# codeslake/RefVSR

Measured on AMD Instinct MI355X. Metric: 4x SR frames/sec (270p->1080p, RefVSR_small_L1), higher is better.
Workload: dtype f16; 1 GPU; config_RefVSR_small_L1 4x SR, 270x480 -> 1080x1920, frame_num=5, steady-state sliding window, n=1 (BASELINE configs[1]); synthetic clip seed 0, seeded random weights 1234; frames_per_rank=20, parallelism=frame-shard x1 (reset-aligned, no collective), window_cache=True, frame_ids=True, pipelined_calls=True, frames_per_call=4, headline_mode=frame groups, pipe_layout=pfm, full=False

## Files before the change

refvsr_amd/csrc/common.h:

```cpp
#pragma once
#include <stdlib.h>
#include <hip/hip_runtime.h>
#include <hip/hip_fp16.h>
#include <stdint.h>
#include <stdio.h>
#include <string.h>
#include <type_traits>
#include <utility>

#include "../../include/refvsr_hip.h"
#include "plan_common.h"

typedef _Float16 f16;
typedef f16 f16x2 __attribute__((ext_vector_type(2)));
typedef f16 f16x4 __attribute__((ext_vector_type(4)));
typedef f16 f16x8 __attribute__((ext_vector_type(8)));
typedef float f32x4 __attribute__((ext_vector_type(4)));
typedef float f32x16 __attribute__((ext_vector_type(16)));

#define RV_HIP(call)                                                                  \
    do {                                                                              \
        hipError_t e_ = (call);                                                       \
        if (e_ != hipSuccess) {                                                       \
            refvsr_set_error("%s failed: %s (%s:%d)", #call, hipGetErrorString(e_), __FILE__, __LINE__); \
// ... 54 lines not shown
    return 0;
}

template <typename Args, typename Launch>
static int rv_resblock_chain(const char* name, int pxb, int min_blob, const void* const* src, int batch, int h, int w, int n,
                             const void* blobs, size_t blob_stride, float act_slope, void* scratch0, void* scratch1, void* const* out,
                             void* stream, Launch launch) {
    RV_CHECK(src && out && blobs && h > 0 && w > 0 && n >= 1 && batch >= 1 && batch <= REFVSR_MAX_MAPS, "%s: bad args", name);
    RV_CHECK(blob_stride >= (size_t)min_blob && blob_stride % 16 == 0 && ((uintptr_t)blobs & 15) == 0,
             "%s: blobs must be 16-byte aligned, stride >= %d", name, min_blob);
    RV_CHECK(act_slope >= 0.f && act_slope <= 1.f, "%s: activation slope must lie in [0, 1]", name);
    RV_CHECK(n == 1 || scratch0, "%s: n >= 2 needs scratch0", name);
    RV_CHECK(n <= 2 || scratch1, "%s: n >= 3 needs scratch1", name);
    const size_t mapb = (size_t)h * w * pxb;
    for (int b = 0; b < batch; ++b) {
        RV_CHECK(src[b] && out[b], "%s: null map pointer (map %d)", name, b);
        for (int c = 0; c < batch; ++c) {
            const unsigned char* s0 = scratch0 ? (const unsigned char*)scratch0 + c * mapb : nullptr;
            const unsigned char* s1 = scratch1 ? (const unsigned char*)scratch1 + c * mapb : nullptr;
            RV_CHECK(src[b] != out[c] && s0 != out[b] && s1 != out[b] && (n < 2 || s0 != src[b]) && (n < 3 || s1 != src[b]) &&
                     (c == b || out[b] != out[c]), "%s: buffers must be distinct", name);
        }
    }
    RV_CHECK(n < 3 || scratch0 != scratch1, "%s: buffers must be distinct", name);
    RV_CHECK((long long)h * w * pxb < (1ll << 31), "%s: map too large for 32-bit offsets", name);
    RV_CHECK(refvsr_init() == 0, "init failed");
    Args a;
    memset(&a, 0, sizeof(a));
    a.h = h; a.w = w; a.act_slope = act_slope; a.batch = batch;
    hipStream_t st = (hipStream_t)stream;
    const unsigned char* cur[REFVSR_MAX_MAPS];
    for (int b = 0; b < batch; ++b) cur[b] = (const unsigned char*)src[b];
    for (int i = 0; i < n; ++i) {
        unsigned char* sc = (unsigned char*)((i & 1) ? scratch1 : scratch0);
        for (int b = 0; b < batch; ++b) {
            a.bsrc[b] = cur[b];
            a.bout[b] = (i == n - 1) ? (unsigned char*)out[b] : sc + b * mapb;
        }
        a.src = a.bsrc[0]; a.out = a.bout[0]; a.blob = (const unsigned char*)blobs + (size_t)i * blob_stride;
        const int rc = launch(a, st);
        if (rc) return rc;
        for (int b = 0; b < batch; ++b) cur[b] = a.bout[b];
    }
    return 0;
}

__device__ __forceinline__ void rv_tile_range(const int n_tiles, const int g, int& t_begin, int& t_end) {
    const int b = (int)blockIdx.x;
    int rank = b;
    if (g >= 8) {
        const int xcd = b & 7;
        rank = b >> 3;
        for (int y = 0; y < xcd; ++y) rank += (g - y + 7) >> 3;
    }
    const unsigned un = (unsigned)n_tiles, ug = (unsigned)g;
    t_begin = (int)(((unsigned)rank * un) / ug);
    t_end = (int)(((unsigned)(rank + 1) * un) / ug);
}

__device__ __forceinline__ int rv_reflect(int i, int n) {
    i = i < 0 ? -i : i;
    return i >= n ? 2 * (n - 1) - i : i;
}

__device__ __forceinline__ float rv_lrelu(float v, float slope) { return v >= 0.f ? v : v * slope; }

__device__ __forceinline__ float rv_linspace_m1p1(int j, int n) {
    const float step = 2.0f / (float)(n - 1);
    return (j < n / 2) ? (-1.0f + step * (float)j) : (1.0f - step * (float)(n - 1 - j));
}

struct WarpCoord { int x0, y0; float w00, w01, w10, w11; bool v00, v01, v10, v11; };

__device__ __forceinline__ WarpCoord warp_coord_uv(const float u, const float v, int hf, int wf, int hin, int win, int y, int x);
__device__ __forceinline__ WarpCoord warp_coord(const float* flow, int hf, int wf, int hin, int win, int y, int x) {
    const size_t fp = (size_t)y * wf + x;
    return warp_coord_uv(flow[fp], flow[(size_t)hf * wf + fp], hf, wf, hin, win, y, x);
}
__device__ __forceinline__ WarpCoord warp_coord_uv(const float u, const float v, int hf, int wf, int hin, int win, int y, int x) {
    const float gx = rv_linspace_m1p1(x, wf) + u / (((float)win - 1.0f) / 2.0f);
    const float gy = rv_linspace_m1p1(y, hf) + v / (((float)hin - 1.0f) / 2.0f);
    const float xs = ((gx + 1.0f) * (float)win - 1.0f) / 2.0f;
    const float ys = ((gy + 1.0f) * (float)hin - 1.0f) / 2.0f;
    const float fx = floorf(xs), fy = floorf(ys);
    const float tx = xs - fx, ty = ys - fy;
    WarpCoord c;
    c.x0 = (int)fminf(fmaxf(fx, -2.0f), (float)win + 1.0f);
    c.y0 = (int)fminf(fmaxf(fy, -2.0f), (float)hin + 1.0f);
    const bool xin0 = c.x0 >= 0 && c.x0 < win, xin1 = c.x0 + 1 >= 0 && c.x0 + 1 < win;
    const bool yin0 = c.y0 >= 0 && c.y0 < hin, yin1 = c.y0 + 1 >= 0 && c.y0 + 1 < hin;
    c.v00 = xin0 && yin0; c.v01 = xin1 && yin0; c.v10 = xin0 && yin1; c.v11 = xin1 && yin1;
    c.w00 = (1.0f - ty) * (1.0f - tx); c.w01 = (1.0f - ty) * tx;
    c.w10 = ty * (1.0f - tx); c.w11 = ty * tx;
    return c;
}

__device__ __forceinline__ uint4 warp_group16(const unsigned char* x, int pixb, int hin, int win, const WarpCoord& c, int goff) {
    float acc[8] = {0, 0, 0, 0, 0, 0, 0, 0};
    auto tap = [&](bool valid, int yy, int xx, float wgt) {
        if (valid) {
            const f16x8 v = *reinterpret_cast<const f16x8*>(x + ((size_t)yy * win + xx) * pixb + goff);
#pragma unroll
            for (int k = 0; k < 8; ++k) acc[k] += wgt * (float)v[k];
        }
    };
    tap(c.v00, c.y0, c.x0, c.w00);
    tap(c.v01, c.y0, c.x0 + 1, c.w01);
    tap(c.v10, c.y0 + 1, c.x0, c.w10);
    tap(c.v11, c.y0 + 1, c.x0 + 1, c.w11);
    union { f16x8 h; uint4 u; } o;
#pragma unroll
    for (int k = 0; k < 8; ++k) o.h[k] = (f16)acc[k];
    return o.u;
}

__device__ __forceinline__ void rv_bilinear_ac_src(int o, int n_in, int n_out, int& i0, int& i1, float& l1) {
#pragma clang fp contract(off)
    const float sc = n_out > 1 ? (float)(n_in - 1) / (float)(n_out - 1) : 0.0f;
    const float x = (float)o * sc;
    i0 = min((int)x, n_in - 1);
    i1 = min(i0 + 1, n_in - 1);
    l1 = x - (float)i0;
}
__device__ __forceinline__ float rv_bilinear_ac2_at(const float* __restrict__ s, int h, int w, int oy, int ox) {
    int y0, y1, x0, x1;
    float ly, lx;
    rv_bilinear_ac_src(oy, h, 2 * h, y0, y1, ly);
    rv_bilinear_ac_src(ox, w, 2 * w, x0, x1, lx);
    const float wy0 = 1.0f - ly, wx0 = 1.0f - lx;
    const float r0 = fmaf(lx, s[(size_t)y0 * w + x1], fmaf(wx0, s[(size_t)y0 * w + x0], 0.0f));
    const float r1 = fmaf(lx, s[(size_t)y1 * w + x1], fmaf(wx0, s[(size_t)y1 * w + x0], 0.0f));
    return fmaf(ly, r1, fmaf(wy0, r0, 0.0f));
}

__device__ __forceinline__ void rv_cubic_taps(float t, float* wgt) {
    const float A = -0.75f;
    float x = t + 1.0f;
    wgt[0] = ((A * x - 5.0f * A) * x + 8.0f * A) * x - 4.0f * A;
    x = t;
    wgt[1] = ((A + 2.0f) * x - (A + 3.0f)) * x * x + 1.0f;
    x = 1.0f - t;
    wgt[2] = ((A + 2.0f) * x - (A + 3.0f)) * x * x + 1.0f;
    x = 2.0f - t;
    wgt[3] = ((A * x - 5.0f * A) * x + 8.0f * A) * x - 4.0f * A;
}
__device__ __forceinline__ void rv_cubic_src(int o, int n_in, float scale, int* idx, float* wgt) {
    const float x = ((float)o + 0.5f) * scale - 0.5f;
    const float fl = floorf(x);
    const int ix = (int)fl;
    rv_cubic_taps(x - fl, wgt);
#pragma unroll
    for (int k = 0; k < 4; ++k) idx[k] = min(max(ix - 1 + k, 0), n_in - 1);
}
__device__ __forceinline__ float rv_bicubic_at(const float* __restrict__ s, int h, int w, int oy, int ox, float sy, float sx) {
    int iy[4], ix[4];
    float wy[4], wx[4];
    rv_cubic_src(oy, h, sy, iy, wy);
    rv_cubic_src(ox, w, sx, ix, wx);
    float acc = 0.0f;
#pragma unroll
    for (int j = 0; j < 4; ++j) {
        float r = 0.0f;
        const float* row = s + (size_t)iy[j] * w;
#pragma unroll
        for (int i = 0; i < 4; ++i) r = fmaf(wx[i], row[ix[i]], r);
        acc = fmaf(wy[j], r, acc);
    }
    return acc;
}

__device__ __forceinline__ void rv_store_result(void* out, const size_t e, const float v, const int fmt) {
    const int f = fmt & REFVSR_RESULT_FMT_MASK;
    if (f == REFVSR_RESULT_F32) reinterpret_cast<float*>(out)[e] = v;
    else if (f == REFVSR_RESULT_F16) reinterpret_cast<f16*>(out)[e] = (f16)v;
    else reinterpret_cast<unsigned char*>(out)[e] = (unsigned char)__float2int_rn(v * 255.0f);
}
__host__ __device__ __forceinline__ size_t rv_result_index(const int fmt, const int c, const int y, const int x, const int h, const int w) {
    return (fmt & REFVSR_RESULT_HWC) ? ((size_t)y * w + x) * 3 + c : ((size_t)c * h + y) * w + x;
}
static inline bool rv_result_fmt_ok(const int fmt) {
    return fmt >= 0 && (fmt & ~(REFVSR_RESULT_FMT_MASK | REFVSR_RESULT_HWC)) == 0 && (fmt & REFVSR_RESULT_FMT_MASK) <= REFVSR_RESULT_U8;
}

__device__ __forceinline__ float rv_fold1(const float a) {
    const unsigned u = __float_as_uint(a);
    const auto pr = __builtin_amdgcn_permlane32_swap(u, u, false, false);
    const unsigned x0 = pr[0], x1 = pr[1];
    return __uint_as_float(x0) + __uint_as_float(x1);
}

__device__ __forceinline__ int rv_pix16(int n) { return (n < 4 || n >= 12) ? ((n & 7) << 1) : (((n - 4) << 1) | 1); }
```

refvsr_amd/csrc/conv24.hip:

```cpp
#include "common.h"
#include "fixed_plan.h"

struct C24Args {
    const unsigned char* src0; const unsigned char* src1; unsigned char* out;
    const unsigned char* blob; const unsigned char* mul; const unsigned char* res;
    int h, w, tiles_x, n_tiles, grid;
    float act_slope, post_slope;
    const float* conf_a; const float* conf_b;
    const float* cw0; const float* cb0;
    float* conf_max;
    int ch, cw;
    float slope0;
    const float* base_lr; int bh, bw; float base_step;
    int out_fmt;
    int batch, tpm;
    const unsigned char* bsrc0[REFVSR_MAX_MAPS]; const unsigned char* bsrc1[REFVSR_MAX_MAPS]; unsigned char* bout[REFVSR_MAX_MAPS];
    const unsigned char* bmul[REFVSR_MAX_MAPS]; const unsigned char* bres[REFVSR_MAX_MAPS];
    const float* bconf_a[REFVSR_MAX_MAPS]; const float* bconf_b[REFVSR_MAX_MAPS]; float* bconf_max[REFVSR_MAX_MAPS];
};

template <int COUT, int NCG0, int NCG1, int NWV, int TH, int WPS, int SHUF = 0, int CONF = 0, int HALF = 0, int MM = 0, int WF = 0>
__global__ __launch_bounds__(NWV * 64) __attribute__((amdgpu_waves_per_eu(WPS, WPS))) void conv24_kernel(C24Args p) {
    static_assert(WF == 0 || COUT != 3, "output head: one fragment in either format");
    static_assert(HALF == 0 || (COUT == 24 && SHUF == 0 && CONF == 0), "channel-half variant: 24 computed channels per workgroup");
    static_assert(MM == 0 || (HALF == 0 && COUT != 3), "multi-map variant");
    static_assert(SHUF == 0 || (COUT == 48 && (SHUF == 24 || SHUF == 48) && NCG0 * 8 == SHUF && NCG1 == 0), "pixel-shuffle variant");
    static_assert(CONF == 0 || (NCG0 == 2 && NCG1 == 0 && SHUF == 0), "confidence variant: 16-channel single source");
    constexpr int NCG = NCG0 + NCG1, PS = NCG | 1, PXB = PS * 16, ROWB = C24_XW * PXB;
    constexpr int S = c24_steps(NCG), NPAT = c24_npat(NCG);
    constexpr int NF = c24_nf(COUT, WF);
    constexpr int NM = COUT == 24 ? 2 : COUT == 3 ? 1 : COUT / 16;
    constexpr int BIASB = COUT == 48 ? 256 : 128;
    constexpr int WB = S * NF * 1024, BIAS = WB, XT = WB + BIASB;
    constexpr int NT = NWV * 64, T = 2 * TH / NWV;
    constexpr int C24_TH = TH, C24_XH = TH + 2, C24_NPX = C24_XH * C24_XW;
    constexpr int NCH = C24_NPX * NCG, KCH = (NCH + NT - 1) / NT;
    constexpr int PIXB0 = NCG0 * 16, PIXB1 = NCG1 * 16;
    constexpr int OPX = HALF ? 96 : COUT * 2;
    static_assert((COUT == 3 || COUT == 24 || COUT == 32 || COUT == 48) && S > 0 && T >= 1 && T * NWV == 2 * TH, "unsupported shape");
    static_assert(COUT != 3 || (NCG1 == 0 && SHUF == 0 && CONF == 0), "output head: single source");
    extern __shared__ __attribute__((aligned(16))) unsigned char smem[];

    asm volatile("" :: "s"(p.src0), "s"(p.src1), "s"(p.out), "s"(p.blob), "s"(p.mul), "s"(p.res), "s"(p.h), "s"(p.w), "s"(p.tiles_x),
                 "s"(p.n_tiles), "s"(p.grid), "s"(p.act_slope), "s"(p.post_slope));
    const int tid = threadIdx.x;
    const int lane = tid & 63;
    const int wave = __builtin_amdgcn_readfirstlane(tid >> 6);

    {
        constexpr int NPC = WB / 1024;
        const unsigned char* g = p.blob + ((SHUF || HALF) ? (int)blockIdx.y * (WB + BIASB) : 0) + lane * 16;
#pragma unroll
        for (int j = 0; j < (NPC + NWV - 1) / NWV; ++j) {
            const int c = wave + j * NWV;
            if (c < NPC)
                __builtin_amdgcn_global_load_lds((const __attribute__((address_space(1))) void*)(g + c * 1024),
                                                 (__attribute__((address_space(3))) void*)(smem + c * 1024), 16, 0, 0);
        }
        if (wave == NPC % NWV && lane < BIASB / 16)
            __builtin_amdgcn_global_load_lds((const __attribute__((address_space(1))) void*)(g + NPC * 1024),
                                             (__attribute__((address_space(3))) void*)(smem + NPC * 1024), 16, 0, 0);
    }

    if constexpr (HALF != 0) {
        const int zoff = (int)blockIdx.y * 48;
        p.out += zoff;
        if (p.mul) p.mul += zoff;
        if (p.res) p.res += zoff;
    }
    const int rowp = p.w;
    unsigned xg[KCH], xl[KCH];
    unsigned xs1 = 0;
#pragma unroll
    for (int k = 0; k < KCH; ++k) {
        const int i = min(tid + k * NT, NCH - 1);
        const int px = i / NCG, cg = i - px * NCG;
        const int r = px / C24_XW, c = px - r * C24_XW;
        const bool s1 = cg >= NCG0;
        xg[k] = (unsigned)((r * rowp + c) * (s1 ? PIXB1 : PIXB0) + (s1 ? cg - NCG0 : cg) * 16);
        xl[k] = (unsigned)(XT + px * PXB + cg * 16);
        xs1 |= s1 ? (1u << k) : 0u;
    }
    uint4 xv[KCH];
    auto x_fetch = [&](const int tf) {
        int t = tf;
        const unsigned char* s0p = p.src0;
        const unsigned char* s1p = p.src1;
        if constexpr (MM != 0) {
            const int bm = (int)((unsigned)tf / (unsigned)p.tpm);
            t = tf - bm * p.tpm;
            s0p = p.bsrc0[bm];
            if constexpr (NCG1 != 0) s1p = p.bsrc1[bm];
        }
        const int tyi = t / p.tiles_x;
        const int ty0 = tyi * C24_TH, tx0 = (t - tyi * p.tiles_x) * C24_TW;
        const bool interior = ty0 >= 1 && ty0 + C24_TH + 1 <= p.h && tx0 >= 1 && tx0 + C24_TW + 1 <= p.w;
        const long long org = (long long)(ty0 - 1) * p.w + (tx0 - 1);
        const unsigned char* b0 = s0p + org * PIXB0;
        const unsigned char* b1 = NCG1 ? s1p + org * PIXB1 : b0;
        if (interior) {
#pragma unroll
            for (int k = 0; k < KCH; ++k)
                xv[k] = *reinterpret_cast<const uint4*>((NCG1 && ((xs1 >> k) & 1) ? b1 : b0) + xg[k]);
        } else {
            int tide = tid;
            asm volatile("" : "+v"(tide));
#pragma unroll
            for (int k = 0; k < KCH; ++k) {
                const int i = min(tide + k * NT, NCH - 1);
                const int px = i / NCG, cg = i - px * NCG;
                const int r = px / C24_XW, c = px - r * C24_XW;
                const int iy = ty0 - 1 + r, ix = tx0 - 1 + c;
                const bool ok = (unsigned)iy < (unsigned)p.h && (unsigned)ix < (unsigned)p.w;
                const bool s1 = cg >= NCG0;
                const unsigned pix = (unsigned)(min(max(iy, 0), p.h - 1) * p.w + min(max(ix, 0), p.w - 1));
                const unsigned char* g = s1 ? s1p + pix * PIXB1 + (cg - NCG0) * 16 : s0p + pix * PIXB0 + cg * 16;
                uint4 v = *reinterpret_cast<const uint4*>(g);
                const unsigned keep = ok ? 0xffffffffu : 0u;
                v.x &= keep; v.y &= keep; v.z &= keep; v.w &= keep;
                xv[k] = v;
            }
        }
    };
    auto x_park = [&]() {
#pragma unroll
        for (int k = 0; k < KCH; ++k)
            if (k * NT + NT <= NCH || tid + k * NT < NCH) *reinterpret_cast<uint4*>(smem + xl[k]) = xv[k];
    };
    constexpr int PTH = TH + 4, PTW = C24_XW + 2;
    constexpr int PT = XT + C24_NPX * PXB, CW0 = PT + 2 * PTH * PTW * 4, CB0 = CW0 + 18 * 16 * 4;
    if constexpr (CONF != 0) {
        float* wl0 = reinterpret_cast<float*>(smem + CW0);
        for (int i = tid; i < 18 * 16; i += NT) {
            const int co = i & 15, tap = i >> 4;
            wl0[i] = p.cw0[(co * 2 + tap / 9) * 9 + tap % 9];
        }
        if (tid < 16) reinterpret_cast<float*>(smem + CB0)[tid] = p.cb0[tid];
    }
    auto conf_stage = [&](const int tf) {
        int t = tf;
        const float* cap = p.conf_a;
        const float* cbp = p.conf_b;
        float* cmp_ = p.conf_max;
        if constexpr (MM != 0) {
            const int bm = (int)((unsigned)tf / (unsigned)p.tpm);
            t = tf - bm * p.tpm;
            cap = p.bconf_a[bm]; cbp = p.bconf_b[bm];
            if (p.conf_max) cmp_ = p.bconf_max[bm];
        }
        const int tyi = t / p.tiles_x;
        const int ty0 = tyi * C24_TH, tx0 = (t - tyi * p.tiles_x) * C24_TW;
        float* pt = reinterpret_cast<float*>(smem + PT);
        for (int i = tid; i < 2 * PTH * PTW; i += NT) {
            const int c = i / (PTH * PTW), rem = i - c * (PTH * PTW);
            const int r = rem / PTW, cc = rem - r * PTW;
            const int y = ty0 - 2 + r, x = tx0 - 2 + cc;
            float v = 0.0f;
            if ((unsigned)y < (unsigned)p.h && (unsigned)x < (unsigned)p.w) {
                const float* src = c ? cbp : cap;
                if constexpr (CONF == 1) v = src[(size_t)y * p.cw + x];
                else v = fminf(fmaxf(rv_bicubic_at(src, p.ch, p.cw, y, x, 0.5f, 0.5f), 0.0f), 1.0f);
            }
            pt[i] = v;
        }
        __syncthreads();
        const float* wl0 = reinterpret_cast<const float*>(smem + CW0);
        const float* bl0 = reinterpret_cast<const float*>(smem + CB0);
#pragma unroll
        for (int k = 0; k < KCH; ++k) {
            const int i = tid + k * NT;
            if (i < NCH) {
                const int px = i >> 1, cg = i & 1;
                const int r = px / C24_XW, c = px - r * C24_XW;
                const int iy = ty0 - 1 + r, ix = tx0 - 1 + c;
                uint4 v = make_uint4(0u, 0u, 0u, 0u);
                if ((unsigned)iy < (unsigned)p.h && (unsigned)ix < (unsigned)p.w) {
                    float acc[8] = {0.f, 0.f, 0.f, 0.f, 0.f, 0.f, 0.f, 0.f};
#pragma unroll
                    for (int ci = 0; ci < 2; ++ci)
#pragma unroll
                        for (int ky = 0; ky < 3; ++ky)
#pragma unroll
                            for (int kx = 0; kx < 3; ++kx) {
                                const float xv = pt[ci * (PTH * PTW) + (r + ky) * PTW + (c + kx)];
                                const f32x4 w0 = *reinterpret_cast<const f32x4*>(wl0 + (ci * 9 + ky * 3 + kx) * 16 + cg * 8);
                                const f32x4 w1 = *reinterpret_cast<const f32x4*>(wl0 + (ci * 9 + ky * 3 + kx) * 16 + cg * 8 + 4);
                                acc[0] = fmaf(xv, w0[0], acc[0]); acc[1] = fmaf(xv, w0[1], acc[1]);
                                acc[2] = fmaf(xv, w0[2], acc[2]); acc[3] = fmaf(xv, w0[3], acc[3]);
                                acc[4] = fmaf(xv, w1[0], acc[4]); acc[5] = fmaf(xv, w1[1], acc[5]);
                                acc[6] = fmaf(xv, w1[2], acc[6]); acc[7] = fmaf(xv, w1[3], acc[7]);
                            }
                    union { f16x8 h; uint4 u; } o;
#pragma unroll
                    for (int j = 0; j < 8; ++j) o.h[j] = (f16)rv_lrelu(acc[j] + bl0[cg * 8 + j], p.slope0);
                    v = o.u;
                }
                *reinterpret_cast<uint4*>(smem + XT + px * PXB + cg * 16) = v;
            }
        }
        if constexpr (CONF == 1) {
            if (p.conf_max) {
                for (int i = tid; i < C24_TH * C24_TW; i += NT) {
                    const int r = i / C24_TW, c = i - r * C24_TW;
                    const int y = ty0 + r, x = tx0 + c;
                    if (y < p.h && x < p.w)
                        cmp_[(size_t)y * p.w + x] = fmaxf(pt[(r + 2) * PTW + c + 2], pt[PTH * PTW + (r + 2) * PTW + c + 2]);
                }
            }
        }
    };
    int tl, k_hi;
    rv_tile_range(p.n_tiles, p.grid, tl, k_hi);
    if constexpr (CONF == 0) { if (tl < k_hi) x_fetch(tl); }
    __builtin_amdgcn_sched_barrier(0);

    const int q = lane >> 4;
    const int lp = rv_pix16(lane & 15);
    const int la = lane * 16;
    const int g0w = wave * T;
#define RW(t) ((g0w + (t)) >> 1)
#define CG(t) ((g0w + (t)) & 1)
    auto sel4 = [&](const int v0, const int v1, const int v2, const int v3) { return q == 0 ? v0 : q == 1 ? v1 : q == 2 ? v2 : v3; };
    int pb[T];
#pragma unroll
    for (int t = 0; t < T; ++t)
        pb[t] = XT + RW(t) * ROWB + (CG(t) * 16 + lp) * PXB +
                sel4(c24_off(NCG, 0, 0), c24_off(NCG, 0, 1), c24_off(NCG, 0, 2), c24_off(NCG, 0, 3)) - c24_off(NCG, 0, 0);
    int pd[NPAT];
#pragma unroll
    for (int pp = 0; pp < NPAT; ++pp) {
        const int s = c24_pat_step(NCG, pp);
        pd[pp] = (sel4(c24_off(NCG, s, 0), c24_off(NCG, s, 1), c24_off(NCG, s, 2), c24_off(NCG, s, 3)) - c24_off(NCG, s, 0)) -
                 (sel4(c24_off(NCG, 0, 0), c24_off(NCG, 0, 1), c24_off(NCG, 0, 2), c24_off(NCG, 0, 3)) - c24_off(NCG, 0, 0));
    }
    const int rowb_o = p.w * OPX;
    const unsigned oo = (unsigned)(lp * OPX + q * 8);

    if constexpr (CONF == 0) { if (tl < k_hi) x_park(); }
    __syncthreads();

    for (; tl < k_hi; ++tl) {
        const bool has_next = tl + 1 < k_hi;
        if constexpr (CONF != 0) {
            conf_stage(tl);
            __syncthreads();
        }
        int tm = tl;
        unsigned char* outp = p.out;
        const unsigned char* mulp = p.mul;
        const unsigned char* resp = p.res;
        if constexpr (MM != 0) {
            const int bm = (int)((unsigned)tl / (unsigned)p.tpm);
            tm = tl - bm * p.tpm;
            outp = p.bout[bm];
            if (p.mul) mulp = p.bmul[bm];
            if (p.res) resp = p.bres[bm];
        }
        const int tyi = tm / p.tiles_x;
        const int ty0 = tyi * C24_TH, tx0 = (tm - tyi * p.tiles_x) * C24_TW;
        const bool interior = ty0 >= 1 && ty0 + C24_TH + 1 <= p.h && tx0 >= 1 && tx0 + C24_TW + 1 <= p.w;
        const long long oorg = ((long long)ty0 * p.w + tx0) * OPX;
        f16x4 mv[NM][T], rv[NM][T];
        bool okt[T];
#pragma unroll
        for (int t = 0; t < T; ++t) {
            okt[t] = true;
            if (!interior) {
                int lpe = lp;
                asm volatile("" : "+v"(lpe));
                okt[t] = ty0 + RW(t) < p.h && tx0 + CG(t) * 16 + lpe < p.w;
            }
            const unsigned eo = (unsigned)(RW(t) * rowb_o) + oo + CG(t) * 16 * OPX;
#pragma unroll
            for (int m = 0; m < NM; ++m) {
                mv[m][t] = rv[m][t] = (f16x4){(f16)0.f, (f16)0.f, (f16)0.f, (f16)0.f};
                const bool lane_ok = okt[t] && (COUT != 24 || m == 0 || q < 2);
                if constexpr (COUT == 24) {
                    if (p.mul && lane_ok) mv[m][t] = *reinterpret_cast<const f16x4*>(mulp + oorg + eo + 32 * m);
                    if (p.res && lane_ok) rv[m][t] = *reinterpret_cast<const f16x4*>(resp + oorg + eo + 32 * m);
                }
                (void)lane_ok;
            }
        }
        if constexpr (CONF == 0) { if (has_next) x_fetch(tl + 1); }

        f32x4 acc[NM][T];
#pragma unroll
        for (int m = 0; m < NM; ++m) {
            const f32x4 bv = *reinterpret_cast<const f32x4*>(smem + BIAS + m * 64 + q * 16);
#pragma unroll
            for (int t = 0; t < T; ++t) acc[m][t] = bv;
        }
        {
            uint4 fa[2][NF], fb[2][T];
            auto load = [&](auto sc, uint4 (&af)[NF], uint4 (&bf)[T]) {
                constexpr int s = decltype(sc)::value;
                constexpr int pp = c24_pat(NCG, s);
                constexpr int imm = c24_off(NCG, s, 0);
#pragma unroll
                for (int f = 0; f < NF; ++f) af[f] = *reinterpret_cast<const uint4*>(smem + (s * NF + f) * 1024 + la);
#pragma unroll
                for (int t = 0; t < T; ++t) {
                    if constexpr (pp == 0) bf[t] = *reinterpret_cast<const uint4*>(smem + pb[t] + imm);
                    else bf[t] = *reinterpret_cast<const uint4*>(smem + pb[t] + pd[pp] + imm);
                }
            };
            auto mfma = [&](const uint4 (&af)[NF], const uint4 (&bf)[T]) {
                if constexpr (WF == 1) {
#pragma unroll
                    for (int m = 0; m < NM; ++m) {
                        const f16x8 av = *reinterpret_cast<const f16x8*>(&af[m]);
#pragma unroll
                        for (int t = 0; t < T; ++t)
                            acc[m][t] = __builtin_amdgcn_mfma_f32_16x16x32_f16(av, *reinterpret_cast<const f16x8*>(&bf[t]), acc[m][t], 0, 0, 0);
                    }
                } else if constexpr (COUT == 24) {
                    const f16x8 a_hi = *reinterpret_cast<const f16x8*>(&af[0]);
                    const f16x8 a_lo = *reinterpret_cast<const f16x8*>(&af[1]);
                    const f16x8 a_mx = *reinterpret_cast<const f16x8*>(&af[2]);
#pragma unroll
                    for (int t = 0; t < T; ++t) acc[0][t] = __builtin_amdgcn_mfma_f32_16x16x32_f16(a_hi, *reinterpret_cast<const f16x8*>(&bf[t]), acc[0][t], 0, 0, 0);
#pragma unroll
                    for (int t = 0; t < T; ++t) acc[1][t] = __builtin_amdgcn_mfma_f32_16x16x32_f16(a_mx, *reinterpret_cast<const f16x8*>(&bf[t]), acc[1][t], 0, 0, 0);
#pragma unroll
                    for (int t = 0; t < T; ++t) acc[0][t] = __builtin_amdgcn_mfma_f32_16x16x32_f16(a_lo, *reinterpret_cast<const f16x8*>(&bf[t]), acc[0][t], 0, 0, 0);
                } else if constexpr (COUT == 3) {
                    const f16x8 a_w = *reinterpret_cast<const f16x8*>(&af[0]);
#pragma unroll
                    for (int t = 0; t < T; ++t) acc[0][t] = __builtin_amdgcn_mfma_f32_16x16x32_f16(a_w, *reinterpret_cast<const f16x8*>(&bf[t]), acc[0][t], 0, 0, 0);
                } else {
#pragma unroll
                    for (int h = 0; h < 2; ++h)
#pragma unroll
                        for (int m = 0; m < NM; ++m) {
                            const f16x8 av = *reinterpret_cast<const f16x8*>(&af[2 * m + h]);
#pragma unroll
                            for (int t = 0; t < T; ++t)
                                acc[m][t] = __builtin_amdgcn_mfma_f32_16x16x32_f16(av, *reinterpret_cast<const f16x8*>(&bf[t]), acc[m][t], 0, 0, 0);
                        }
                }
            };
            if constexpr (NF <= 4) {
                load(std::integral_constant<int, 0>{}, fa[0], fb[0]);
                rv_static_for([&](auto sc) {
                    constexpr int s = decltype(sc)::value;
                    if constexpr (s + 1 < S) load(std::integral_constant<int, s + 1>{}, fa[(s + 1) & 1], fb[(s + 1) & 1]);
                    __builtin_amdgcn_sched_barrier(0);
                    mfma(fa[s & 1], fb[s & 1]);
                }, std::make_integer_sequence<int, S>{});
            } else {
                load(std::integral_constant<int, 0>{}, fa[0], fb[0]);
                rv_static_for([&](auto sc) {
                    constexpr int s = decltype(sc)::value;
                    __builtin_amdgcn_sched_barrier(0);
                    mfma(fa[0], fb[0]);
                    __builtin_amdgcn_sched_barrier(0);
                    if constexpr (s + 1 < S) load(std::integral_constant<int, s + 1>{}, fa[0], fb[0]);
                }, std::make_integer_sequence<int, S>{});
            }
        }
        if (has_next) {
            __syncthreads();
            if constexpr (CONF == 0) x_park();
        }
        if constexpr (COUT == 3) {
            const size_t plane_b = (size_t)p.bh * p.bw;
#pragma unroll
            for (int t = 0; t < T; ++t) {
                const f32x4 y = acc[0][t];
                const float s0 = rv_fold1(y[0]), s1 = rv_fold1(y[1]), s2 = rv_fold1(y[2]);
                const int srcl = lane & 15;
                const float v0 = __shfl(s0, srcl), v1 = __shfl(s1, srcl), v2 = __shfl(s2, srcl);
                const float v = q == 0 ? v0 : q == 1 ? v1 : v2;
                int lpe = lp;
                if (!interior) asm volatile("" : "+v"(lpe));
                const int oy = ty0 + RW(t), ox = tx0 + CG(t) * 16 + lpe;
                if (q < 3 && oy < p.h && ox < p.w) {
                    const float b = fminf(fmaxf(rv_bicubic_at(p.base_lr + q * plane_b, p.bh, p.bw, oy, ox, p.base_step, p.base_step), 0.0f), 1.0f);
                    rv_store_result(outp, rv_result_index(p.out_fmt, q, oy, ox, p.h, p.w), fminf(fmaxf(v + b, 0.0f), 1.0f), p.out_fmt);
                }
            }
        } else if constexpr (SHUF != 0) {
            const int z = (int)blockIdx.y;
            const unsigned w2 = 2u * (unsigned)p.w;
#pragma unroll
            for (int t = 0; t < T; ++t) {
                int lpe = lp;
                if (!interior) asm volatile("" : "+v"(lpe));
                const unsigned oy = (unsigned)(ty0 + RW(t)), ox = (unsigned)(tx0 + CG(t) * 16 + lpe);
#pragma unroll
                for (int m = 0; m < NM; ++m) {
                    const int r0 = 16 * m + 4 * q;
                    const int dx = SHUF == 24 ? (r0 >= 24 ? 1 : 0) : (z & 1);
                    const int dy = SHUF == 24 ? z : (z >> 1);
                    const int ch0 = SHUF == 24 ? r0 - 24 * dx : r0;
                    f32x4 y = acc[m][t];
                    if (p.act_slope != 1.0f) {
#pragma unroll
                        for (int i = 0; i < 4; ++i) y[i] = fmaxf(y[i], y[i] * p.act_slope);
                    }
                    const f16x4 o = {(f16)y[0], (f16)y[1], (f16)y[2], (f16)y[3]};
                    if (okt[t])
                        *reinterpret_cast<f16x4*>(outp + ((2u * oy + dy) * w2 + 2u * ox + dx) * (unsigned)(SHUF * 2) + ch0 * 2) = o;
                }
            }
        } else
        {
            unsigned char* ob = outp + oorg;
#pragma unroll
            for (int t = 0; t < T; ++t) {
                unsigned char* d = ob + (unsigned)(RW(t) * rowb_o) + oo + CG(t) * 16 * OPX;
#pragma unroll
                for (int m = 0; m < NM; ++m) {
                    f32x4 y = acc[m][t];
                    if constexpr (COUT == 24) {
                        if (WF == 0 && m == 1) y = (f32x4){rv_fold1(y[0]), rv_fold1(y[1]), rv_fold1(y[2]), rv_fold1(y[3])};
                    } else {
                        const unsigned eo = (unsigned)(RW(t) * rowb_o) + oo + CG(t) * 16 * OPX;
                        if (p.mul && okt[t]) mv[m][t] = *reinterpret_cast<const f16x4*>(mulp + oorg + eo + 32 * m);
                        if (p.res && okt[t]) rv[m][t] = *reinterpret_cast<const f16x4*>(resp + oorg + eo + 32 * m);
                    }
                    if (p.act_slope != 1.0f) {
#pragma unroll
                        for (int i = 0; i < 4; ++i) y[i] = fmaxf(y[i], y[i] * p.act_slope);
                    }
                    if (p.mul) {
#pragma unroll
                        for (int i = 0; i < 4; ++i) y[i] *= (float)mv[m][t][i];
                    }
                    if (p.res) {
#pragma unroll
                        for (int i = 0; i < 4; ++i) y[i] += (float)rv[m][t][i];
                    }
                    if (p.post_slope != 1.0f) {
#pragma unroll
                        for (int i = 0; i < 4; ++i) y[i] = fmaxf(y[i], y[i] * p.post_slope);
                    }
                    const f16x4 o = {(f16)y[0], (f16)y[1], (f16)y[2], (f16)y[3]};
                    if (okt[t] && (COUT != 24 || m == 0 || q < 2)) *reinterpret_cast<f16x4*>(d + 32 * m) = o;
                }
            }
        }
        if constexpr (CONF == 0) { if (has_next) __syncthreads(); }
    }
#undef RW
#undef CG
}

template <int COUT, int NCG0, int NCG1, int NWV, int TH, int WPS, int SHUF, int CONF, int HALF, int MM, int WF>
static int launch_c24(C24Args& a, const C24Plan& p, hipStream_t st) {
    constexpr int NZ = c24_nz(SHUF, HALF), LDS = c24_lds(COUT, NCG0 + NCG1, TH, CONF, WF);
    static_assert(LDS <= 160 * 1024, "LDS budget");
    static RvLaunchCap lc = {};
    int cap;
    if (int rc = rv_launch_cap(lc, &conv24_kernel<COUT, NCG0, NCG1, NWV, TH, WPS, SHUF, CONF, HALF, MM, WF>, NWV * 64, LDS, LDS, st, &cap, NZ)) return rc;
    a.tiles_x = p.tiles_x; a.tpm = p.tpm; a.n_tiles = p.n_tiles;
    a.grid = a.n_tiles < cap ? a.n_tiles : cap;
    hipLaunchKernelGGL((conv24_kernel<COUT, NCG0, NCG1, NWV, TH, WPS, SHUF, CONF, HALF, MM, WF>), dim3(a.grid, NZ), dim3(NWV * 64), LDS, st, a);
    RV_LAUNCH_CHECK();
    return 0;
}

static const C24Knobs& c24_knobs() {
    static const C24Knobs knobs = c24_knobs_from_env();
    return knobs;
}

static const char* c24_no_kernel(const C24Plan& p) { return p.no_twin ? p.no_twin : "conv24: no kernel for this plan"; }

static int c24_dispatch(C24Args& a, const C24Plan& p, void* stream) {
    switch (p.key()) {
#define RV_C24_CASE(...) case c24_variant_key(__VA_ARGS__): return launch_c24<__VA_ARGS__>(a, p, (hipStream_t)stream);
        RV_C24_VARIANTS(RV_C24_CASE)
#undef RV_C24_CASE
    }
    RV_CHECK(false, "%s", c24_no_kernel(p));
    return 1;
}

extern "C" int refvsr_conv24_variant(int op, int x0, int x1, int mm, int wf, int batch, int h, int w, long long* key, int* n_tiles, int* lds) {
    RV_CHECK(key != nullptr, "conv24_variant: null key");
    RV_CHECK(op >= C24_CONV24 && op <= C24_CONV_LAST && (mm == 0 || mm == 1) && (wf == 0 || wf == 1) && h > 0 && w > 0, "conv24_variant: bad args");
    C24Plan p;
    if (int rc = c24_plan((C24Op)op, x0, x1, mm, wf, mm ? batch : 1, h, w, c24_knobs(), &p)) return rc;
    bool listed = false;
    switch (p.key()) {
#define RV_C24_CASE(...) case c24_variant_key(__VA_ARGS__):
        RV_C24_VARIANTS(RV_C24_CASE) listed = !p.no_twin;
#undef RV_C24_CASE
    }
    RV_CHECK(listed, "%s", c24_no_kernel(p));
    *key = p.key();
    if (n_tiles) *n_tiles = p.n_tiles;
    if (lds) *lds = p.lds;
    return 0;
}

extern "C" int refvsr_conv24_supported(int c0, int c1) { return c24_supported(C24_CONV24, c0, c1); }
extern "C" int refvsr_conv48_supported(int c0, int c1) { return c24_supported(C24_CONV48, c0, c1); }
extern "C" int refvsr_conv32_supported(int c0, int c1) { return c24_supported(C24_CONV32, c0, c1); }
extern "C" int refvsr_conv_shuffle2_supported(int c) { return c24_supported(C24_SHUFFLE2, c, 0); }

extern "C" int refvsr_conv24_blob_bytes(int c0, int c1) { return refvsr_conv24_supported(c0, c1) ? c24_blob_bytes(24, (c0 + c1) / 8, 0) : -1; }
extern "C" int refvsr_conv32_blob_bytes(int c0, int c1) { return refvsr_conv32_supported(c0, c1) ? c24_blob_bytes(32, (c0 + c1) / 8, 0) : -1; }
extern "C" int refvsr_conv48_blob_bytes(int c0, int c1) {
    if (!refvsr_conv48_supported(c0, c1)) return -1;
    return c0 == 48 && c1 == 48 ? c24_nz(0, 1) * c24_blob_bytes(24, 12, 0) : c24_blob_bytes(48, (c0 + c1) / 8, 0);
}
extern "C" int refvsr_conv_shuffle2_blob_bytes(int c) { return refvsr_conv_shuffle2_supported(c) ? c24_nz(c, 0) * c24_blob_bytes(48, c / 8, 0) : -1; }
extern "C" int refvsr_conv24_f16w_blob_bytes(int c0, int c1) { return refvsr_conv24_supported(c0, c1) ? c24_blob_bytes(24, (c0 + c1) / 8, 1) : -1; }
extern "C" int refvsr_conv32_f16w_blob_bytes(int c0, int c1) { return refvsr_conv32_supported(c0, c1) ? c24_blob_bytes(32, (c0 + c1) / 8, 1) : -1; }
extern "C" int refvsr_conv_shuffle2_f16w_blob_bytes(int c) { return c == 24 ? c24_nz(c, 0) * c24_blob_bytes(48, c / 8, 1) : -1; }

extern "C" int refvsr_conv24_kblock(int ncg, int s, int q) {
    if (c24_steps(ncg) == 0 || s < 0 || s >= c24_steps(ncg) || q < 0 || q > 3) return -2;
    return c24_kblock(ncg, s, q);
}

static int c24_fill(C24Args& a, const char* who, int cout, const void* src0, const void* src1, int c1, int h, int w, const void* blob,
                    float act_slope, const void* mul, const void* res, float post_slope, void* out) {
    RV_CHECK(src0 && out && blob && h > 0 && w > 0, "%s: bad args", who);
    RV_CHECK((c1 == 0) == (src1 == nullptr), "%s: src1 / c1 mismatch", who);
    RV_CHECK(((uintptr_t)blob & 15) == 0, "%s: blob must be 16-byte aligned", who);
    RV_CHECK(act_slope >= 0.f && act_slope <= 1.f && post_slope >= 0.f && post_slope <= 1.f, "%s: activation slopes must lie in [0, 1]", who);
    RV_CHECK(src0 != out && src1 != out, "%s: in-place operation is not supported", who);
    RV_CHECK((long long)h * w * cout * 2 < (1ll << 31), "%s: map too large for 32-bit offsets", who);
    RV_CHECK(refvsr_init() == 0, "init failed");
    memset(&a, 0, sizeof(a));
    a.src0 = (const unsigned char*)src0; a.src1 = (const unsigned char*)src1; a.out = (unsigned char*)out;
    a.blob = (const unsigned char*)blob; a.mul = (const unsigned char*)mul; a.res = (const unsigned char*)res;
    a.h = h; a.w = w; a.act_slope = act_slope; a.post_slope = post_slope;
    return 0;
}

static int c24_fill_maps(C24Args& a, const char* who, int cout, const void* const* src0, const void* const* src1, int c1, int batch,
                         int h, int w, const void* blob, float act_slope, const void* const* mul, const void* const* res,
                         float post_slope, void* const* out) {
    if (c24_fill(a, who, cout, src0[0], src1 ? src1[0] : nullptr, c1, h, w, blob, act_slope, mul ? mul[0] : nullptr,
                 res ? res[0] : nullptr, post_slope, out[0])) return 1;
    a.batch = batch;
    for (int b = 0; b < batch; ++b) {
        RV_CHECK(src0[b] && out[b] && (!src1 || src1[b]) && (!mul || mul[b]) && (!res || res[b]), "%s: null map pointer (map %d)", who, b);
        for (int c = 0; c < batch; ++c)
            RV_CHECK(src0[c] != out[b] && (!src1 || src1[c] != out[b]) && (c == b || out[c] != out[b]), "%s: in-place operation is not supported", who);
        a.bsrc0[b] = (const unsigned char*)src0[b]; a.bsrc1[b] = src1 ? (const unsigned char*)src1[b] : nullptr;
        a.bout[b] = (unsigned char*)out[b];
        a.bmul[b] = mul ? (const unsigned char*)mul[b] : nullptr; a.bres[b] = res ? (const unsigned char*)res[b] : nullptr;
    }
    return 0;
}
#define C24_OPT(p) ((p) ? &(p) : nullptr)

static int c24_conv24(int wf, int mm, const void* const* src0, int c0, const void* const* src1, int c1, int batch, int h, int w, const void* blob,
                      float act_slope, const void* const* mul, const void* const* res, float post_slope, void* const* out, void* stream) {
    const char* who = mm ? "conv24_batch" : "conv24";
    C24Plan p;
    C24Args a;
    if (c24_plan(C24_CONV24, c0, c1, mm, wf, batch, h, w, c24_knobs(), &p)) return 1;
    RV_CHECK(src0 && out, "%s: 1..%d maps per launch", who, REFVSR_MAX_MAPS);
    RV_CHECK(!mm || (c1 == 0) == (src1 == nullptr), "%s: src1 / c1 mismatch", who);
    if (c24_fill_maps(a, who, 24, src0, src1, c1, batch, h, w, blob, act_slope, mul, res, post_slope, out)) return 1;
    return c24_dispatch(a, p, stream);
}
#define C24_CONV_ARGS const void* src0, int c0, const void* src1, int c1, int h, int w, const void* blob, float act_slope, \
                      const void* mul, const void* res, float post_slope, void* out, void* stream
#define C24_CONV_BATCH_ARGS const void* const* src0, int c0, const void* const* src1, int c1, int batch, int h, int w, const void* blob, \
                            float act_slope, const void* const* mul, const void* const* res, float post_slope, void* const* out, void* stream
#define C24_CONV_PASS(WF) c24_conv24(WF, 0, &src0, c0, C24_OPT(src1), c1, 1, h, w, blob, act_slope, C24_OPT(mul), C24_OPT(res), post_slope, &out, stream)
#define C24_CONV_BATCH_PASS(WF) c24_conv24(WF, 1, src0, c0, src1, c1, batch, h, w, blob, act_slope, mul, res, post_slope, out, stream)
extern "C" int refvsr_conv24(C24_CONV_ARGS) { return C24_CONV_PASS(0); }
extern "C" int refvsr_conv24_f16w(C24_CONV_ARGS) { return C24_CONV_PASS(1); }
extern "C" int refvsr_conv24_batch(C24_CONV_BATCH_ARGS) { return C24_CONV_BATCH_PASS(0); }
extern "C" int refvsr_conv24_batch_f16w(C24_CONV_BATCH_ARGS) { return C24_CONV_BATCH_PASS(1); }

static int c24_conv_single(C24Op op, const char* who, int cout, int wf, C24_CONV_ARGS) {
    C24Plan p;
    C24Args a;
    if (c24_plan(op, c0, c1, 0, wf, 1, h, w, c24_knobs(), &p)) return 1;
    if (c24_fill(a, who, cout, src0, src1, c1, h, w, blob, act_slope, mul, res, post_slope, out)) return 1;
    return c24_dispatch(a, p, stream);
}
#define C24_CONV_SINGLE(OP, WHO, COUT, WF) c24_conv_single(OP, WHO, COUT, WF, src0, c0, src1, c1, h, w, blob, act_slope, mul, res, post_slope, out, stream)
extern "C" int refvsr_conv32(C24_CONV_ARGS) { return C24_CONV_SINGLE(C24_CONV32, "conv32", 32, 0); }
extern "C" int refvsr_conv32_f16w(C24_CONV_ARGS) { return C24_CONV_SINGLE(C24_CONV32, "conv32", 32, 1); }
extern "C" int refvsr_conv48(C24_CONV_ARGS) { return C24_CONV_SINGLE(C24_CONV48, "conv48", 48, 0); }

static int c24_conv_shuffle2(int wf, int mm, const void* const* src, int batch, int c, int h, int w, const void* blobs, float act_slope,
                             void* const* out, void* stream) {
    const char* who = mm ? "conv_shuffle2_batch" : "conv_shuffle2";
    C24Plan p;
    C24Args a;
    if (c24_plan(C24_SHUFFLE2, c, 0, mm, wf, batch, h, w, c24_knobs(), &p)) return 1;
    RV_CHECK(src && out, "%s: 1..%d maps per launch", who, REFVSR_MAX_MAPS);
    if (c24_fill_maps(a, who, 4 * c, src, nullptr, 0, batch, h, w, blobs, act_slope, nullptr, nullptr, 1.0f, out)) return 1;
    return c24_dispatch(a, p, stream);
}
// ... 60 lines not shown
```

Baseline: 236.4 frames/s.

## Prefetch confidence inputs across tiles and factor bicubic upsample in conv24 confidence stage

The confidence variant of the fused conv24 kernel now prefetches the raw confidence window for the next tile into registers during the current tile's MMA work, then parks it in LDS. The bicubic 2x upsample reuses separable row sums with fixed even/odd tap weights instead of a full 16-tap evaluation per output. The first-layer 2->16 conv is restructured so each thread computes a run of 3 pixels by 4 output channels with double-buffered operand loads. The changes aim to hide global-load latency and cut redundant interpolation and LDS traffic, at the cost of more registers and extra barriers per tile in the confidence path.

```diff
diff --git a/refvsr_amd/csrc/common.h b/refvsr_amd/csrc/common.h
--- a/refvsr_amd/csrc/common.h
+++ b/refvsr_amd/csrc/common.h
@@ -230,21 +230,23 @@
 #pragma unroll
     for (int k = 0; k < 4; ++k) idx[k] = min(max(ix - 1 + k, 0), n_in - 1);
 }
+template <class F>
+__device__ __forceinline__ float rv_cubic_dot(const float* wgt, F v) {
+    float r = 0.0f;
+#pragma unroll
+    for (int k = 0; k < 4; ++k) r = fmaf(wgt[k], v(k), r);
+    return r;
+}
+template <class F>
+__device__ __forceinline__ float rv_bicubic_eval(const float* wy, const float* wx, F tap) {
+    return rv_cubic_dot(wy, [&](const int j) { return rv_cubic_dot(wx, [&](const int i) { return tap(j, i); }); });
+}
 __device__ __forceinline__ float rv_bicubic_at(const float* __restrict__ s, int h, int w, int oy, int ox, float sy, float sx) {
     int iy[4], ix[4];
     float wy[4], wx[4];
     rv_cubic_src(oy, h, sy, iy, wy);
     rv_cubic_src(ox, w, sx, ix, wx);
-    float acc = 0.0f;
-#pragma unroll
-    for (int j = 0; j < 4; ++j) {
-        float r = 0.0f;
-        const float* row = s + (size_t)iy[j] * w;
-#pragma unroll
-        for (int i = 0; i < 4; ++i) r = fmaf(wx[i], row[ix[i]], r);
-        acc = fmaf(wy[j], r, acc);
-    }
-    return acc;
+    return rv_bicubic_eval(wy, wx, [&](const int j, const int i) { return (s + (size_t)iy[j] * w)[ix[i]]; });
 }
 
 __device__ __forceinline__ void rv_store_result(void* out, const size_t e, const float v, const int fmt) {
diff --git a/refvsr_amd/csrc/conv24.hip b/refvsr_amd/csrc/conv24.hip
--- a/refvsr_amd/csrc/conv24.hip
+++ b/refvsr_amd/csrc/conv24.hip
@@ -137,70 +137,156 @@
         }
         if (tid < 16) reinterpret_cast<float*>(smem + CB0)[tid] = p.cb0[tid];
     }
-    auto conf_stage = [&](const int tf) {
+    constexpr int RWH = TH / 2 + 6, RWW = C24_TW / 2 + 6, RWS = (RWW + 3) / 4;
+    constexpr int NRAW = CONF == 2 ? 2 * RWH * RWW : 2 * PTH * PTW, KRAW = (NRAW + NT - 1) / NT;
+    static_assert(CONF == 0 || (PS == 3 && 2 * RWH * RWS <= C24_NPX && TH % 2 == 0), "confidence variant: raw window in slot 2 of the x tile");
+    auto raw_off = [](const int c, const int r, const int cc) { return XT + 32 + ((c * RWH + r) * RWS + (cc >> 2)) * PXB + (cc & 3) * 4; };
+    float craw[KRAW];
+    unsigned cok = 0;
+    auto conf_fetch = [&](const int tf) {
+        int tide = tid;
+        asm volatile("" : "+v"(tide));
         int t = tf;
         const float* cap = p.conf_a;
         const float* cbp = p.conf_b;
+        if constexpr (MM != 0) {
+            const int bm = (int)((unsigned)tf / (unsigned)p.tpm);
+            t = tf - bm * p.tpm;
+            cap = p.bconf_a[bm]; cbp = p.bconf_b[bm];
+        }
+        const int tyi = t / p.tiles_x;
+        const int ty0 = tyi * C24_TH, tx0 = (t - tyi * p.tiles_x) * C24_TW;
+        cok = 0;
+#pragma unroll
+        for (int k = 0; k < KRAW; ++k) {
+            const int i = min(tide + k * NT, NRAW - 1);
+            if constexpr (CONF == 1) {
+                const int c = i / (PTH * PTW), rem = i - c * (PTH * PTW);
+                const int r = rem / PTW, cc = rem - r * PTW;
+                const int y = ty0 - 2 + r, x = tx0 - 2 + cc;
+                cok |= ((unsigned)y < (unsigned)p.h && (unsigned)x < (unsigned)p.w) ? (1u << k) : 0u;
+                craw[k] = (c ? cbp : cap)[(size_t)min(max(y, 0), p.h - 1) * p.cw + min(max(x, 0), p.w - 1)];
+            } else {
+                const int c = i / (RWH * RWW), rem = i - c * (RWH * RWW);
+                const int r = rem / RWW, cc = rem - r * RWW;
+                const int y = min(max(ty0 / 2 - 3 + r, 0), p.ch - 1), x = min(max(tx0 / 2 - 3 + cc, 0), p.cw - 1);
+                craw[k] = (c ? cbp : cap)[(size_t)y * p.cw + x];
+            }
+        }
+    };
+    auto conf_park = [&]() {
+        int tide = tid;
+        asm volatile("" : "+v"(tide));
+#pragma unroll
+        for (int k = 0; k < KRAW; ++k) {
+            const int i = tide + k * NT;
+            if (k * NT + NT <= NRAW || i < NRAW) {
+                if constexpr (CONF == 1) {
+                    reinterpret_cast<float*>(smem + PT)[i] = ((cok >> k) & 1) ? craw[k] : 0.0f;
+                } else {
+                    const int c = i / (RWH * RWW), rem = i - c * (RWH * RWW);
+                    const int r = rem / RWW, cc = rem - r * RWW;
+                    *reinterpret_cast<float*>(smem + raw_off(c, r, cc)) = craw[k];
+                }
+            }
+        }
+    };
+    auto conf_stage = [&](const int tf) {
+        int tide = tid;
+        asm volatile("" : "+v"(tide));
+        int t = tf;
         float* cmp_ = p.conf_max;
         if constexpr (MM != 0) {
             const int bm = (int)((unsigned)tf / (unsigned)p.tpm);
             t = tf - bm * p.tpm;
-            cap = p.bconf_a[bm]; cbp = p.bconf_b[bm];
             if (p.conf_max) cmp_ = p.bconf_max[bm];
         }
         const int tyi = t / p.tiles_x;
         const int ty0 = tyi * C24_TH, tx0 = (t - tyi * p.tiles_x) * C24_TW;
         float* pt = reinterpret_cast<float*>(smem + PT);
-        for (int i = tid; i < 2 * PTH * PTW; i += NT) {
-            const int c = i / (PTH * PTW), rem = i - c * (PTH * PTW);
-            const int r = rem / PTW, cc = rem - r * PTW;
-            const int y = ty0 - 2 + r, x = tx0 - 2 + cc;
-            float v = 0.0f;
-            if ((unsigned)y < (unsigned)p.h && (unsigned)x < (unsigned)p.w) {
-                const float* src = c ? cbp : cap;
-                if constexpr (CONF == 1) v = src[(size_t)y * p.cw + x];
-                else v = fminf(fmaxf(rv_bicubic_at(src, p.ch, p.cw, y, x, 0.5f, 0.5f), 0.0f), 1.0f);
-            }
-            pt[i] = v;
-        }
-        __syncthreads();
+        if constexpr (CONF == 2) {
+            float wev[4], wod[4];
+            rv_cubic_taps(0.75f, wev);
+            rv_cubic_taps(0.25f, wod);
+            if (tide < PTH * PTW) {
+                const int c = tide / (PTH / 2 * PTW), rem = tide - c * (PTH / 2 * PTW);
+                const int k = rem / PTW, cc = rem - k * PTW;
+                const int y = ty0 - 2 + 2 * k, x = tx0 - 2 + cc, rx = (cc + 1) >> 1;
+                float wx[4];
+#pragma unroll
+                for (int i = 0; i < 4; ++i) wx[i] = (cc & 1) ? wod[i] : wev[i];
+                int co[4];
+#pragma unroll
+                for (int i = 0; i < 4; ++i) co[i] = raw_off(0, 0, rx + i) - raw_off(0, 0, 0);
+                float rs[5];
+#pragma unroll
+                for (int j = 0; j < 5; ++j) {
+                    const unsigned char* row = smem + raw_off(c, k + j, 0);
+                    rs[j] = rv_cubic_dot(wx, [&](const int i) { return *reinterpret_cast<const float*>(row + co[i]); });
+                }
+                float v0 = rv_cubic_dot(wev, [&](const int j) { return rs[j]; });
+                float v1 = rv_cubic_dot(wod, [&](const int j) { return rs[j + 1]; });
+                const bool xin = (unsigned)x < (unsigned)p.w;
+                v0 = (xin && (unsigned)y < (unsigned)p.h) ? fminf(fmaxf(v0, 0.0f), 1.0f) : 0.0f;
+                v1 = (xin && (unsigned)(y + 1) < (unsigned)p.h) ? fminf(fmaxf(v1, 0.0f), 1.0f) : 0.0f;
+                pt[c * (PTH * PTW) + 2 * k * PTW + cc] = v0;
+                pt[c * (PTH * PTW) + (2 * k + 1) * PTW + cc] = v1;
+            }
+            __syncthreads();
+        }
         const float* wl0 = reinterpret_cast<const float*>(smem + CW0);
         const float* bl0 = reinterpret_cast<const float*>(smem + CB0);
-#pragma unroll
-        for (int k = 0; k < KCH; ++k) {
-            const int i = tid + k * NT;
-            if (i < NCH) {
-                const int px = i >> 1, cg = i & 1;
-                const int r = px / C24_XW, c = px - r * C24_XW;
-                const int iy = ty0 - 1 + r, ix = tx0 - 1 + c;
-                uint4 v = make_uint4(0u, 0u, 0u, 0u);
-                if ((unsigned)iy < (unsigned)p.h && (unsigned)ix < (unsigned)p.w) {
-                    float acc[8] = {0.f, 0.f, 0.f, 0.f, 0.f, 0.f, 0.f, 0.f};
-#pragma unroll
-                    for (int ci = 0; ci < 2; ++ci)
-#pragma unroll
-                        for (int ky = 0; ky < 3; ++ky)
-#pragma unroll
-                            for (int kx = 0; kx < 3; ++kx) {
-                                const float xv = pt[ci * (PTH * PTW) + (r + ky) * PTW + (c + kx)];
-                                const f32x4 w0 = *reinterpret_cast<const f32x4*>(wl0 + (ci * 9 + ky * 3 + kx) * 16 + cg * 8);
-                                const f32x4 w1 = *reinterpret_cast<const f32x4*>(wl0 + (ci * 9 + ky * 3 + kx) * 16 + cg * 8 + 4);
-                                acc[0] = fmaf(xv, w0[0], acc[0]); acc[1] = fmaf(xv, w0[1], acc[1]);
-                                acc[2] = fmaf(xv, w0[2], acc[2]); acc[3] = fmaf(xv, w0[3], acc[3]);
-                                acc[4] = fmaf(xv, w1[0], acc[4]); acc[5] = fmaf(xv, w1[1], acc[5]);
-                                acc[6] = fmaf(xv, w1[2], acc[6]); acc[7] = fmaf(xv, w1[3], acc[7]);
-                            }
-                    union { f16x8 h; uint4 u; } o;
-#pragma unroll
-                    for (int j = 0; j < 8; ++j) o.h[j] = (f16)rv_lrelu(acc[j] + bl0[cg * 8 + j], p.slope0);
-                    v = o.u;
-                }
-                *reinterpret_cast<uint4*>(smem + XT + px * PXB + cg * 16) = v;
+        constexpr int RUN = 3, NRUN = (C24_XW + RUN - 1) / RUN;
+        static_assert(CONF == 0 || C24_XH * NRUN * 4 <= NT, "stage 2: one work item per thread");
+        const int it = tide >> 2, cog = tide & 3;
+        if (it < C24_XH * NRUN) {
+            const int r = it / NRUN, c0 = min((it - r * NRUN) * RUN, C24_XW - RUN);
+            float acc[RUN][4];
+#pragma unroll
+            for (int j = 0; j < RUN; ++j)
+#pragma unroll
+                for (int o = 0; o < 4; ++o) acc[j][o] = 0.0f;
+            float xw[2][RUN + 2];
+            f32x4 wv[2][3];
+            const float* ptr = pt + r * PTW;
+            const float* wlc = wl0 + cog * 4;
+            auto rd = [&](auto gc, float (&xr)[RUN + 2], f32x4 (&wr)[3]) {
+                constexpr int g = decltype(gc)::value, ci = g / 3, ky = g - 3 * ci;
+#pragma unroll
+                for (int d = 0; d < RUN + 2; ++d) xr[d] = ptr[ci * (PTH * PTW) + ky * PTW + c0 + d];
+#pragma unroll
+                for (int kx = 0; kx < 3; ++kx) wr[kx] = *reinterpret_cast<const f32x4*>(wlc + (g * 3 + kx) * 16);
+            };
+            rd(std::integral_constant<int, 0>{}, xw[0], wv[0]);
+            rv_static_for([&](auto gc) {
+                constexpr int g = decltype(gc)::value;
+                if constexpr (g + 1 < 6) rd(std::integral_constant<int, g + 1>{}, xw[(g + 1) & 1], wv[(g + 1) & 1]);
+                __builtin_amdgcn_sched_barrier(0);
+#pragma unroll
+                for (int kx = 0; kx < 3; ++kx)
+#pragma unroll
+                    for (int j = 0; j < RUN; ++j) {
+                        const float xv = xw[g & 1][j + kx];
+                        const f32x4 w = wv[g & 1][kx];
+                        acc[j][0] = fmaf(xv, w[0], acc[j][0]); acc[j][1] = fmaf(xv, w[1], acc[j][1]);
+                        acc[j][2] = fmaf(xv, w[2], acc[j][2]); acc[j][3] = fmaf(xv, w[3], acc[j][3]);
+                    }
+            }, std::make_integer_sequence<int, 6>{});
+            const f32x4 bv = *reinterpret_cast<const f32x4*>(bl0 + cog * 4);
+            const int iy = ty0 - 1 + r;
+#pragma unroll
+            for (int j = 0; j < RUN; ++j) {
+                const int c = c0 + j, ix = tx0 - 1 + c;
+                union { f16x4 h; uint2 u; } o;
+#pragma unroll
+                for (int e = 0; e < 4; ++e) o.h[e] = (f16)rv_lrelu(acc[j][e] + bv[e], p.slope0);
+                const unsigned keep = ((unsigned)iy < (unsigned)p.h && (unsigned)ix < (unsigned)p.w) ? 0xffffffffu : 0u;
+                *reinterpret_cast<uint2*>(smem + XT + (r * C24_XW + c) * PXB + cog * 8) = make_uint2(o.u.x & keep, o.u.y & keep);
             }
         }
         if constexpr (CONF == 1) {
             if (p.conf_max) {
-                for (int i = tid; i < C24_TH * C24_TW; i += NT) {
+                for (int i = tide; i < C24_TH * C24_TW; i += NT) {
                     const int r = i / C24_TW, c = i - r * C24_TW;
                     const int y = ty0 + r, x = tx0 + c;
                     if (y < p.h && x < p.w)
@@ -211,7 +297,10 @@
     };
     int tl, k_hi;
     rv_tile_range(p.n_tiles, p.grid, tl, k_hi);
-    if constexpr (CONF == 0) { if (tl < k_hi) x_fetch(tl); }
+    if (tl < k_hi) {
+        if constexpr (CONF == 0) x_fetch(tl);
+        else conf_fetch(tl);
+    }
     __builtin_amdgcn_sched_barrier(0);
 
     const int q = lane >> 4;
@@ -236,11 +325,15 @@
     const int rowb_o = p.w * OPX;
     const unsigned oo = (unsigned)(lp * OPX + q * 8);
 
-    if constexpr (CONF == 0) { if (tl < k_hi) x_park(); }
+    if (tl < k_hi) {
+        if constexpr (CONF == 0) x_park();
+        else conf_park();
+    }
     __syncthreads();
 
     for (; tl < k_hi; ++tl) {
         const bool has_next = tl + 1 < k_hi;
+        const bool use_mul = CONF == 0 && p.mul, use_res = CONF == 0 && p.res;
         if constexpr (CONF != 0) {
             conf_stage(tl);
             __syncthreads();
@@ -253,8 +346,8 @@
             const int bm = (int)((unsigned)tl / (unsigned)p.tpm);
             tm = tl - bm * p.tpm;
             outp = p.bout[bm];
-            if (p.mul) mulp = p.bmul[bm];
-            if (p.res) resp = p.bres[bm];
+            if (use_mul) mulp = p.bmul[bm];
+            if (use_res) resp = p.bres[bm];
         }
         const int tyi = tm / p.tiles_x;
         const int ty0 = tyi * C24_TH, tx0 = (tm - tyi * p.tiles_x) * C24_TW;
@@ -276,13 +369,16 @@
                 mv[m][t] = rv[m][t] = (f16x4){(f16)0.f, (f16)0.f, (f16)0.f, (f16)0.f};
                 const bool lane_ok = okt[t] && (COUT != 24 || m == 0 || q < 2);
                 if constexpr (COUT == 24) {
-                    if (p.mul && lane_ok) mv[m][t] = *reinterpret_cast<const f16x4*>(mulp + oorg + eo + 32 * m);
-                    if (p.res && lane_ok) rv[m][t] = *reinterpret_cast<const f16x4*>(resp + oorg + eo + 32 * m);
+                    if (use_mul && lane_ok) mv[m][t] = *reinterpret_cast<const f16x4*>(mulp + oorg + eo + 32 * m);
+                    if (use_res && lane_ok) rv[m][t] = *reinterpret_cast<const f16x4*>(resp + oorg + eo + 32 * m);
                 }
                 (void)lane_ok;
             }
         }
-        if constexpr (CONF == 0) { if (has_next) x_fetch(tl + 1); }
+        if (has_next) {
+            if constexpr (CONF == 0) x_fetch(tl + 1);
+            else conf_fetch(tl + 1);
+        }
 
         f32x4 acc[NM][T];
 #pragma unroll
@@ -359,9 +455,14 @@
                 }, std::make_integer_sequence<int, S>{});
             }
         }
-        if (has_next) {
-            __syncthreads();
-            if constexpr (CONF == 0) x_park();
+        if constexpr (CONF == 0) {
+            if (has_next) {
+                __syncthreads();
+                x_park();
+            }
+        }
+        else {
+            if (has_next) conf_park();
         }
         if constexpr (COUT == 3) {
             const size_t plane_b = (size_t)p.bh * p.bw;
@@ -417,18 +518,18 @@
                         if (WF == 0 && m == 1) y = (f32x4){rv_fold1(y[0]), rv_fold1(y[1]), rv_fold1(y[2]), rv_fold1(y[3])};
                     } else {
                         const unsigned eo = (unsigned)(RW(t) * rowb_o) + oo + CG(t) * 16 * OPX;
-                        if (p.mul && okt[t]) mv[m][t] = *reinterpret_cast<const f16x4*>(mulp + oorg + eo + 32 * m);
-                        if (p.res && okt[t]) rv[m][t] = *reinterpret_cast<const f16x4*>(resp + oorg + eo + 32 * m);
+                        if (use_mul && okt[t]) mv[m][t] = *reinterpret_cast<const f16x4*>(mulp + oorg + eo + 32 * m);
+                        if (use_res && okt[t]) rv[m][t] = *reinterpret_cast<const f16x4*>(resp + oorg + eo + 32 * m);
                     }
                     if (p.act_slope != 1.0f) {
 #pragma unroll
                         for (int i = 0; i < 4; ++i) y[i] = fmaxf(y[i], y[i] * p.act_slope);
                     }
-                    if (p.mul) {
+                    if (use_mul) {
 #pragma unroll
                         for (int i = 0; i < 4; ++i) y[i] *= (float)mv[m][t][i];
                     }
-                    if (p.res) {
+                    if (use_res) {
 #pragma unroll
                         for (int i = 0; i < 4; ++i) y[i] += (float)rv[m][t][i];
                     }
@@ -441,7 +542,9 @@
                 }
             }
         }
-        if constexpr (CONF == 0) { if (has_next) __syncthreads(); }
+        if (has_next) {
+            __syncthreads();
+        }
     }
 #undef RW
 #undef CG
```

After: 235.7 frames/s. About the same (-0.3%).
